# YuePanEdward/GH-ICP

Measured on AMD Instinct MI355X. Metric: registered_pairs_per_sec, higher is better.
Workload: dtype f64

## Files before the change

### gh-icp_amd/csrc/batch.hip

```cpp
#include "batch_dev.h"
#include "frontend.h"
#include "pca_dev.h"
#include "bsc_dev.h"
#include "prims.h"

#include <cmath>

namespace {

enum { FB_CLOUD_BY_CLOUD = -1, FB_HALVE = -2 };

__global__ void k_fb_bbox_init(int* __restrict__ bb, int nb) {
  const int i = blockIdx.x * 256 + threadIdx.x;
  if (i < nb * 6) bb[i] = (i % 6) < 3 ? 0x7f7fffff : (int)0x80800000;
}

__global__ __launch_bounds__(256) void k_fb_bbox(const FbBlock* __restrict__ D, const float* __restrict__ base, int which, int* __restrict__ bb) {
  __shared__ float smin[3][4], smax[3][4];
  const int b = blockIdx.y;
  const float* xyz;
  long long n;
  int stride;
  if (which == 0) { xyz = D->c[b].xyz; n = D->c[b].n; stride = D->c[b].stride; }
  else {
// ... 178 lines not shown
  const int b = fb_find(D->moff, D->nb, i);
  D->c[b].ds[i - D->moff[b]] = dsg[i];
}

__global__ __launch_bounds__(256) void k_fb_keypoints_out(const FbBlock* __restrict__ D, const float4* __restrict__ dsg, const int* __restrict__ kpg, int K,
                                                          float* __restrict__ lcs) {
  const int t = blockIdx.x * 256 + threadIdx.x;
  if (t >= K) return;
  const int b = fb_find(D->koff, D->nb, t), j = t - D->koff[b];
  const int id = kpg[D->coff[b] + j];
  const float4 P = dsg[D->moff[b] + id];
  const FbCloud& C = D->c[b];
  C.kp[j] = id;
  C.kpx[(size_t)j * 3] = (double)P.x; C.kpx[(size_t)j * 3 + 1] = (double)P.y; C.kpx[(size_t)j * 3 + 2] = (double)P.z;
  if (lcs) { lcs[(size_t)t * 12 + 9] = P.x; lcs[(size_t)t * 12 + 10] = P.y; lcs[(size_t)t * 12 + 11] = P.z; }
}

__global__ __launch_bounds__(256) void k_fb_zero_feat(const FbBlock* __restrict__ D, int K) {
  const int t = blockIdx.x * 256 + threadIdx.x;
  if (t >= K * 56) return;
  const int q = t / 56, r = t % 56, v = r / 14, w = r % 14;
  const int b = fb_find(D->koff, D->nb, q), j = q - D->koff[b], kb = D->koff[b + 1] - D->koff[b];
  reinterpret_cast<unsigned*>(D->c[b].feat)[((size_t)v * kb + j) * 14 + w] = 0u;
}

__global__ __launch_bounds__(256) void k_fb_gather_rows33(const FbBlock* __restrict__ D, const float* __restrict__ hist, int K) {
  const int t = blockIdx.x * 256 + threadIdx.x;
  if (t >= K * 33) return;
  const int q = t / 33, r = t % 33;
  const int b = fb_find(D->koff, D->nb, q), j = q - D->koff[b];
  reinterpret_cast<float*>(D->c[b].feat)[(size_t)j * 33 + r] = hist[((size_t)D->moff[b] + D->c[b].kp[j]) * 33 + r];
}

__global__ __launch_bounds__(BT) void k_fb_bsc(const FbBlock* __restrict__ D, const float4* __restrict__ pts, const unsigned* __restrict__ start, BscConst C,
                                               float* __restrict__ lcs) {
  const int q = blockIdx.x;
  const int b = fb_find(D->koff, D->nb, q);
  GridArgs G;
  G.d = D->g2[b]; G.pts = pts; G.start = start + D->cb2[b];
  gh_bsc_keypoint(G, C, q - D->koff[b], D->koff[b + 1] - D->koff[b], D->c[b].feat, lcs + (size_t)D->koff[b] * 12);
}

void decode_box(const int* enc, float* mm) {
  for (int k = 0; k < 6; k++) {
    const int i = enc[k] >= 0 ? enc[k] : enc[k] ^ 0x7fffffff;
    memcpy(&mm[k], &i, 4);
  }
}

int build_grid(ghicp_ctx* ctx, const FbBlock* D, int which, const float4* dsg, int M, unsigned total_cells, const GridSlots& sl, const float4** pts_out,
               const unsigned** start_out, const unsigned** keys_out) {
  hipStream_t s = ctx->stream;
  unsigned *keys, *keys2, *vals, *vals2, *start;
  float4* pts;
  GH_TRY(ctx->reserve(sl.keys, (size_t)M + 1, &keys));
  GH_TRY(ctx->reserve(sl.keys2, (size_t)M + 1, &keys2));
  GH_TRY(ctx->reserve(sl.vals, (size_t)M + 1, &vals));
  GH_TRY(ctx->reserve(sl.vals2, (size_t)M + 1, &vals2));
  GH_TRY(ctx->reserve(sl.start, (size_t)total_cells + 2, &start));
  GH_TRY(ctx->reserve(sl.pts, (size_t)M + 1, &pts));
  hipEvent_t kg = ctx->kt_begin(KT_FB_GRID);
  hipLaunchKernelGGL(k_fb_cell_keys, dim3(cdiv(M, 256)), dim3(256), 0, s, D, which, dsg, M, keys, vals);
  GH_TRY(gh_radix_sort_u32(ctx, keys, keys2, vals, vals2, M, 0, bits_for(total_cells)));
  hipLaunchKernelGGL(k_fb_gather_sorted, dim3(cdiv(M, 256)), dim3(256), 0, s, dsg, vals2, M, pts);
  gh_cell_start_launch(s, keys2, (unsigned)M, total_cells, start);
  ctx->kt_end(KT_FB_GRID, kg);
  GH_HIP(hipGetLastError());
  *pts_out = pts; *start_out = start; *keys_out = keys2;
  return GHICP_OK;
}

int fb_cloud_by_cloud(int n_clouds, ghicp_cloud* const* clouds, const float* const* xyz, const int64_t* n, int stride) {
  for (int i = 0; i < n_clouds; i++) GH_TRY(ghicp_cloud_recompute(clouds[i], xyz[i], n[i], stride));
// ... 172 lines not shown
  for (int b = 0; b < nb; b++) clouds[b]->cand = H->coff[b + 1] - H->coff[b];
  Ctot = H->coff[nb];
  return GHICP_OK;
}

int FbRun::outputs() {
  for (int b = 0; b < nb; b++) {
    ghicp_cloud* c = clouds[b];
    GH_HIP(c->ds.reserve(((size_t)c->m + 1) * sizeof(float4)));
    GH_HIP(c->kp.reserve(((size_t)c->m + 1) * sizeof(int)));
    GH_HIP(c->kpx.reserve(((size_t)c->k * 3 + 3) * sizeof(double)));
    if (bsc) GH_HIP(c->feat.reserve((size_t)4 * c->k * 56 + 64));
    if (fpfh) GH_HIP(c->feat.reserve(((size_t)c->k * 33 + 33) * sizeof(float)));
    H->c[b].ds = c->ds.as<float4>(); H->c[b].kp = c->kp.as<int>(); H->c[b].kpx = c->kpx.as<double>(); H->c[b].feat = c->feat.as<uint8_t>();
  }
  GH_HIP(upload());
  hipEvent_t ko = ctx->kt_begin(KT_FB_OUT);
  hipLaunchKernelGGL(k_fb_copy_ds, dim3(cdiv(M, 256)), dim3(256), 0, s, (const FbBlock*)D, (const float4*)dsg, M);
  lcs = nullptr;
  if (Ktot > 0) {
    if (bsc) GH_TRY(ctx->reserve(B_P_LCS, (size_t)Ktot * 12 + 12, &lcs));
    hipLaunchKernelGGL(k_fb_keypoints_out, dim3(cdiv(Ktot, 256)), dim3(256), 0, s, (const FbBlock*)D, (const float4*)dsg, (const int*)kpg, Ktot, lcs);
    if (bsc) hipLaunchKernelGGL(k_fb_zero_feat, dim3(cdiv((long long)Ktot * 56, 256)), dim3(256), 0, s, (const FbBlock*)D, Ktot);
  }
  ctx->kt_end(KT_FB_OUT, ko);
  return GHICP_OK;
}

int FbRun::features(const BscConst& BC) {
  if (Ktot > 0 && (bsc || fpfh)) {
    const float4* pts2;
    const unsigned *start2, *keys2;
    const GridSlots sl2 = {B_GRID2_KEYS, B_GRID2_KEYS2, B_GRID2_VALS, B_GRID2_VALS2, B_GRID2_START, B_GRID2_PTS};
    GH_TRY(build_grid(ctx, D, 1, dsg, M, (unsigned)t2, sl2, &pts2, &start2, &keys2));
    if (bsc) {
      hipEvent_t kb = ctx->kt_begin(KT_BSC);
      hipLaunchKernelGGL(k_fb_bsc, dim3((unsigned)Ktot), dim3(BT), 0, s, (const FbBlock*)D, pts2, start2, BC, lcs);
      ctx->kt_end(KT_BSC, kb);
    } else {
      float* hist;
      GH_TRY(ctx->reserve(B_P_FEAT_S, (size_t)M * 33 * sizeof(float) + 64, (char**)&hist));
      GH_TRY(gh_fpfh_batch_dev(ctx, dsg, M, pts2, start2, D->g2, D->cb2, D->moff, nb, hist));
      hipLaunchKernelGGL(k_fb_gather_rows33, dim3(cdiv((long long)Ktot * 33, 256)), dim3(256), 0, s, (const FbBlock*)D, (const float*)hist, Ktot);
    }
  }
  GH_HIP(hipGetLastError());
  GH_HIP(hipStreamSynchronize(s));
  return GHICP_OK;
}

extern "C" int ghicp_clouds_recompute(ghicp_ctx* ctx, int32_t n_clouds, ghicp_cloud* const* clouds, const float* const* xyz, const int64_t* n, int stride) {
  GH_ENTER(ctx);
  GH_ARG(n_clouds >= 0 && (n_clouds == 0 || (clouds != nullptr && xyz != nullptr && n != nullptr)) && stride >= 3);
  if (n_clouds == 0) return GHICP_OK;
  FbRun R;
  R.ctx = ctx; R.s = ctx->stream; R.nb = n_clouds; R.clouds = clouds; R.N = 0;
  for (int i = 0; i < n_clouds; i++) {
    GH_ARG(clouds[i] != nullptr && clouds[i]->ctx == ctx && n[i] >= 0 && n[i] < (1ll << 31) - 2);
    if (!same_front_end(clouds[i]->cfg, clouds[0]->cfg))
      return ctx->fail(GHICP_ERR_ARG, "ghicp_clouds_recompute: cloud %d has a different front-end configuration", i);
    for (int j = 0; j < i; j++) GH_ARG(clouds[j] != clouds[i]);
    R.N += n[i];
  }
  R.cfg = clouds[0]->cfg; R.bsc = R.cfg.reg.feature == GHICP_FEATURE_BSC; R.fpfh = R.cfg.reg.feature == GHICP_FEATURE_FPFH;
  if (!(R.cfg.voxel > 0.f) || ctx->host_ptrs) return fb_cloud_by_cloud(n_clouds, clouds, xyz, n, stride);
  if (n_clouds > FB_MAX || R.N + n_clouds >= (1ll << 31) - 2) return fb_halve(ctx, n_clouds, clouds, xyz, n, stride);
  GH_TRY(R.begin(xyz, n, stride));
  if (R.N == 0) return GHICP_OK;
  BscConst BC;
  int rc = R.raw_boxes();
  if (rc == GHICP_OK) rc = R.voxel();
// ... 10 lines not shown
```

### gh-icp_amd/csrc/bsc.hip

```cpp
#include "frontend.h"
#include "devmath.h"
#include "bsc_dev.h"

namespace {

__global__ __launch_bounds__(BT) void k_bsc(GridArgs G, const int* __restrict__ kp, BscConst C, uint8_t* __restrict__ feat, float* __restrict__ lcs) {
  gh_bsc_keypoint(G, C, (int)blockIdx.x, C.K, feat, lcs);
}

__global__ __launch_bounds__(256) void k_bsc_origins(const float* __restrict__ xyz, int stride, const int* __restrict__ kp, int K, float* __restrict__ lcs) {
  const int k = blockIdx.x * 256 + threadIdx.x;
  if (k >= K) return;
  const long long s = kp[k];
  lcs[(size_t)k * 12 + 9] = xyz[s * stride];
  lcs[(size_t)k * 12 + 10] = xyz[s * stride + 1];
  lcs[(size_t)k * 12 + 11] = xyz[s * stride + 2];
}

}

int gh_bsc_make_const(ghicp_ctx* ctx, float R, int dof, const int32_t* pattern_host, BscConst* out, float* r_search) {
  BscConst C;
  memset(&C, 0, sizeof(C));
  C.R = R;
  const double rs = std::sqrt(3.0) * (double)R;
  C.r2s = (float)(rs * rs);
  C.u = 2 * R / 7;
  const float delta = (float)(C.u * 0.5);
  C.den = 2 * delta * delta;
  C.r2c = (float)((1.5 * (double)C.u) * (1.5 * (double)C.u));
  C.area = (float)(M_PI * (double)R * (double)R);
  C.radius_w = std::sqrt(2.0) * (double)R;
  int ex = 0;
  (void)std::frexp((double)R * 0.5, &ex);
  C.dunit = std::ldexp(1.0, 24 - ex);
  C.dinv = std::ldexp(1.0, ex - 54);
  for (int i = 0; i < 7; i++) C.centre[i] = (float)((i + 0.5) * (double)C.u - (double)R);
  for (int i = 0; i < 98; i++) {
    C.pattern[i] = pattern_host[i];
    if (C.pattern[i] < 0 || C.pattern[i] > 48) return ctx->fail(GHICP_ERR_ARG, "BSC sample pattern entry %d out of [0,48]", i);
  }
  C.K = 0;
  C.nvar = (dof > 4) ? 4 : (dof > 0 ? 2 : 1);
  *out = C;
  *r_search = (float)rs;
  return GHICP_OK;
}

int gh_bsc_dev(ghicp_ctx* ctx, const float* xyz, long long m, int stride, const int32_t* kp, long long K, float R, int dof, const int32_t* pattern_host,
               uint8_t* feat, float* lcs) {
  if (K <= 0) return GHICP_OK;
  hipStream_t s = ctx->stream;
  BscConst C;
  float r_search_f = 0.f;
  GH_TRY(gh_bsc_make_const(ctx, R, dof, pattern_host, &C, &r_search_f));
  C.K = (int)K;
  DeviceGrid G;
  const GridSlots sl = {B_GRID2_KEYS, B_GRID2_KEYS2, B_GRID2_VALS, B_GRID2_VALS2, B_GRID2_START, B_GRID2_PTS};
  GH_TRY(gh_grid_build(ctx, xyz, m, stride, r_search_f * 1.0001f, sl, &G));
  GH_HIP(hipMemsetAsync(feat, 0, (size_t)4 * K * 56, s));
  hipLaunchKernelGGL(k_bsc_origins, dim3(cdiv(K, 256)), dim3(256), 0, s, xyz, stride, kp, (int)K, lcs);
  GridArgs A = {G.d, G.pts, G.start};
  hipEvent_t kt = ctx->kt_begin(KT_BSC);
  hipLaunchKernelGGL(k_bsc, dim3((unsigned)K), dim3(BT), 0, s, A, kp, C, feat, lcs);
  ctx->kt_end(KT_BSC, kt);
  GH_HIP(hipGetLastError());
  return GHICP_OK;
}

extern "C" int ghicp_bsc_encode(ghicp_ctx* ctx, const float* xyz, int64_t m, int stride, const int32_t* kp_idx, int64_t k, float radius, int dof,
                                const int32_t* pattern, uint8_t* feat, float* lcs) {
  GH_ENTER(ctx);
  GH_ARG(m >= 0 && m < (1ll << 31) - 2 && k >= 0 && k <= m && stride >= 3 && radius > 0.f && pattern != nullptr);
  Stager sg(ctx);
  const float* d;
  const int32_t* dk;
  uint8_t* df;
  float* dl;
  GH_TRY(sg.in_cloud(xyz, (size_t)m * stride, &d));
  GH_TRY(sg.in(kp_idx, (size_t)k, &dk));
  GH_TRY(sg.out(feat, (size_t)4 * k * 56, &df));
  GH_TRY(sg.out(lcs, (size_t)k * 12, &dl));
  GH_TRY(gh_bsc_dev(ctx, d, m, stride, dk, k, radius, dof, pattern, df, dl));
  return sg.finish();
}
```

### gh-icp_amd/csrc/bsc_dev.h

```cpp
#pragma once
#include "grid.h"
#include "devmath.h"
#include "bsc_exp_table.h"

struct BscConst {
  float R, r2s, u, den, r2c, area;
  double radius_w;
  double dunit, dinv;
  float centre[7];
  int pattern[98];
  int K, nvar;
};

constexpr int BT = 256;
constexpr int BSC_CAP = 2048;
constexpr int BSC_CHUNK = 512;

int gh_bsc_make_const(ghicp_ctx* ctx, float R, int dof, const int32_t* pattern_host, BscConst* out, float* r_search);

static __device__ const double gh_bsc_exp_tab[145] = {GH_BSC_EXP_TABLE};
__device__ inline float gh_bsc_expf(float xf, const double* __restrict__ tab) {
  const double x = (double)xf;
  int j = (int)(x * -32.0 + 0.5);
  j = j < 0 ? 0 : (j > 144 ? 144 : j);
  const double s = x + (double)j * 0.03125;
  double p = s * (1.0 / 720.0) + (1.0 / 120.0);
  p = s * p + (1.0 / 24.0);
  p = s * p + (1.0 / 6.0);
  p = s * p + 0.5;
  p = s * p + 1.0;
  p = s * p + 1.0;
  return (float)(tab[j] * p);
}

__device__ inline void gh_bsc_depth_add(unsigned long long* __restrict__ lo64, unsigned* __restrict__ carry, float depth, float ew, double dunit) {
  const unsigned d_off = (unsigned)((int)((double)depth * dunit) + (1 << 27));
  const unsigned w_int = (unsigned)((double)ew * 1073741824.0);
  const unsigned long long term = (unsigned long long)d_off * (unsigned long long)w_int;
  const unsigned long long old = atomicAdd(lo64, term);
  if (old + term < old) atomicAdd(carry, 1u);
}
__device__ inline double gh_bsc_depth_sum(unsigned long long lo64, unsigned carry, double pnum, double dinv) {
  const unsigned __int128 acc = ((unsigned __int128)carry << 64) | (unsigned __int128)lo64;
  const unsigned __int128 shift = (unsigned __int128)(unsigned long long)(pnum * 1073741824.0) << 27;
  const bool neg = acc < shift;
  const unsigned __int128 mag = neg ? shift - acc : acc - shift;
  const double d = (double)(unsigned long long)(mag >> 32) * 4294967296.0 + (double)(unsigned long long)(mag & 0xFFFFFFFFull);
  return (neg ? -d : d) * dinv;
}

__device__ inline int rearr_src(int type, int k) {
  switch (type) {
    case 1: return 48 - k;
    case 2: return (6 - k / 7) * 7 + k % 7;
    default: return (k / 7) * 7 + 6 - k % 7;
  }
}

__device__ inline void gh_bsc_keypoint(const GridArgs& G, const BscConst& C, int kk, int K, uint8_t* __restrict__ feat, float* __restrict__ lcs) {

  __shared__ double red[16];
  __shared__ double s_pnum[147], s_exp[145];
  __shared__ unsigned long long s_dlo[147];
  __shared__ unsigned s_dcarry[147];
  __shared__ float s_weight[147], s_depth[147];
  __shared__ float s_axes[9];
  __shared__ double s_stat[3][4];
  __shared__ unsigned s_bits[4][16];
  __shared__ float4 s_pts[BSC_CHUNK];
  __shared__ int s_scan[17];
  __shared__ float s_centre[8];
  const int tid = threadIdx.x;
  const float qx = lcs[(size_t)kk * 12 + 9], qy = lcs[(size_t)kk * 12 + 10], qz = lcs[(size_t)kk * 12 + 11];
  const int cx = gh_cell_coord(qx, G.d.mn[0], G.d.inv, G.d.dim[0]);
  const int cy = gh_cell_coord(qy, G.d.mn[1], G.d.inv, G.d.dim[1]);
  const int cz = gh_cell_coord(qz, G.d.mn[2], G.d.inv, G.d.dim[2]);

  double sx = 0, sy = 0, sz = 0, sw = 0;
  int cnt = 0;
  gh_for_runs(G.d, G.start, cx, cy, cz, [&](unsigned b, unsigned e) {
    for (unsigned q = b + tid; q < e; q += BT) {
      const float4 P = G.pts[q];
      const float dx = qx - P.x, dy = qy - P.y, dz = qz - P.z;
      float d2 = dx * dx;
      d2 += dy * dy;
      d2 += dz * dz;
      if (d2 < C.r2s) {
        cnt++;
        sx += (double)P.x; sy += (double)P.y; sz += (double)P.z;
        sw += C.radius_w - (double)sqrtf(d2);
      }
    }
  });
  sx = gh_block_sum(sx, red); sy = gh_block_sum(sy, red); sz = gh_block_sum(sz, red); sw = gh_block_sum(sw, red);
  int mm;
  const int my_base = gh_block_excl_scan(cnt, s_scan, &mm);
  const double mx = sx / (double)mm, my = sy / (double)mm, mz = sz / (double)mm;
  const bool packed = mm <= BSC_CAP;
  auto fill_chunk = [&](int c0) {
    int w = my_base;
    gh_for_runs(G.d, G.start, cx, cy, cz, [&](unsigned b, unsigned e) {
      for (unsigned q = b + tid; q < e; q += BT) {
        const float4 P = G.pts[q];
        const float dx = qx - P.x, dy = qy - P.y, dz = qz - P.z;
        float d2 = dx * dx;
        d2 += dy * dy;
        d2 += dz * dz;
        if (d2 < C.r2s) {
          if (w >= c0 && w < c0 + BSC_CHUNK) s_pts[w - c0] = make_float4(P.x, P.y, P.z, d2);
          w++;
        }
      }
    });
    __syncthreads();
  };

  double c00 = 0, c01 = 0, c02 = 0, c11 = 0, c12 = 0, c22 = 0;
  if (mm >= 3 && packed) {
    for (int c0 = 0; c0 < mm; c0 += BSC_CHUNK) {
      fill_chunk(c0);
      const int cn = min(BSC_CHUNK, mm - c0);
      for (int t = tid; t < cn; t += BT) {
        const float4 P = s_pts[t];
        const double w = (double)(float)(C.radius_w - (double)sqrtf(P.w));
        const double ex = (double)P.x - mx, ey = (double)P.y - my, ez = (double)P.z - mz;
        c00 += w * ex * ex; c01 += w * ex * ey; c02 += w * ex * ez;
        c11 += w * ey * ey; c12 += w * ey * ez; c22 += w * ez * ez;
      }
      __syncthreads();
    }
  } else if (mm >= 3) {
    gh_for_runs(G.d, G.start, cx, cy, cz, [&](unsigned b, unsigned e) {
      for (unsigned q = b + tid; q < e; q += BT) {
        const float4 P = G.pts[q];
        const float dx = qx - P.x, dy = qy - P.y, dz = qz - P.z;
        float d2 = dx * dx;
        d2 += dy * dy;
        d2 += dz * dz;
        if (d2 < C.r2s) {
          const double w = (double)(float)(C.radius_w - (double)sqrtf(d2));
          const double ex = (double)P.x - mx, ey = (double)P.y - my, ez = (double)P.z - mz;
          c00 += w * ex * ex; c01 += w * ex * ey; c02 += w * ex * ez;
          c11 += w * ey * ey; c12 += w * ey * ez; c22 += w * ez * ez;
        }
      }
    });
  }
  if (mm >= 3) {
    c00 = gh_block_sum(c00, red); c01 = gh_block_sum(c01, red); c02 = gh_block_sum(c02, red);
    c11 = gh_block_sum(c11, red); c12 = gh_block_sum(c12, red); c22 = gh_block_sum(c22, red);
  }
  if (tid == 0) {
    float X[3] = {1, 0, 0}, Y[3] = {0, 1, 0}, Z[3] = {0, 0, 1};
    if (mm >= 3) {
      const float da = (float)sw;
      double Cq[6] = {c00, c01, c02, c11, c12, c22};
      gh_quant_grid(Cq, 6);
      double a00 = (double)((float)Cq[0] / da), a01 = (double)((float)Cq[1] / da), a02 = (double)((float)Cq[2] / da),
             a11 = (double)((float)Cq[3] / da), a12 = (double)((float)Cq[4] / da), a22 = (double)((float)Cq[5] / da);
      double V[9];
      gh_jacobi3(a00, a01, a02, a11, a12, a22, V);
      const double ev[3] = {a00, a11, a22};
      int imax = 0, imin = 0;
// ... 1 lines not shown
        if ((float)ev[i] > (float)ev[imax]) imax = i;
        if ((float)ev[i] < (float)ev[imin]) imin = i;
      }
      float P[3], N[3];
      for (int which = 0; which < 2; which++) {
        const int col = which == 0 ? imax : imin;
        const double e[3] = {V[0 * 3 + col], V[1 * 3 + col], V[2 * 3 + col]};
        int b = 0;
        if (fabs(e[1]) > fabs(e[b])) b = 1;
        if (fabs(e[2]) > fabs(e[b])) b = 2;
        const double sg = (e[b] < 0) ? -1.0 : 1.0;
        float* o = which == 0 ? P : N;
        for (int d = 0; d < 3; d++) o[d] = (float)(sg * e[d]);
      }
      const float M0 = P[1] * N[2] - P[2] * N[1], M1 = P[2] * N[0] - P[0] * N[2], M2 = P[0] * N[1] - P[1] * N[0];
      X[0] = P[0]; X[1] = P[1]; X[2] = P[2];
      Y[0] = M0; Y[1] = M1; Y[2] = M2;
      Z[0] = X[1] * Y[2] - X[2] * Y[1];
      Z[1] = X[2] * Y[0] - X[0] * Y[2];
      Z[2] = X[0] * Y[1] - X[1] * Y[0];
      const float nx = sqrtf((X[0] * X[0] + X[1] * X[1]) + X[2] * X[2]);
      const float ny = sqrtf((Y[0] * Y[0] + Y[1] * Y[1]) + Y[2] * Y[2]);
      for (int d = 0; d < 3; d++) { X[d] = X[d] / nx; Y[d] = Y[d] / ny; }
    }
    for (int d = 0; d < 3; d++) { s_axes[d] = X[d]; s_axes[3 + d] = Y[d]; s_axes[6 + d] = Z[d]; }
    float* o = &lcs[(size_t)kk * 12];
    for (int d = 0; d < 3; d++) { o[d] = X[d]; o[3 + d] = Y[d]; o[6 + d] = Z[d]; }
  }
  for (int i = tid; i < 147; i += BT) { s_pnum[i] = 0.0; s_dlo[i] = 0ull; s_dcarry[i] = 0u; }
  for (int i = tid; i < 145; i += BT) s_exp[i] = gh_bsc_exp_tab[i];
  if (tid < 7) s_centre[tid] = C.centre[tid];
  if (tid < 64) s_bits[tid >> 4][tid & 15] = 0u;
  __syncthreads();
  const float X0 = s_axes[0], X1 = s_axes[1], X2 = s_axes[2], Y0 = s_axes[3], Y1 = s_axes[4], Y2 = s_axes[5], Z0 = s_axes[6], Z1 = s_axes[7],
              Z2 = s_axes[8];

  auto splat = [&](float px, float py, float pz) {
    const float d0 = px - qx, d1 = py - qy, d2v = pz - qz;
    const float loc[3] = {(X0 * d0 + X1 * d1) + X2 * d2v, (Y0 * d0 + Y1 * d1) + Y2 * d2v, (Z0 * d0 + Z1 * d1) + Z2 * d2v};
#pragma unroll
    for (int pl = 0; pl < 3; pl++) {
      const float a = loc[pl == 2 ? 1 : 0], bb = loc[pl == 0 ? 1 : 2];
      const float depth = loc[pl == 0 ? 2 : (pl == 1 ? 1 : 0)] + C.R;
      for (int j = 0; j < 7; j++) {
        const float dy = bb - C.centre[j];
        const float dy2 = dy * dy;
        if (!(dy2 < C.r2c)) continue;
        for (int i = 0; i < 7; i++) {
          const float dx = a - C.centre[i];
          float dd = dx * dx;
          dd += dy2;
          if (dd < C.r2c) {
            const float ew = gh_bsc_expf(-dd / C.den, s_exp);
            atomicAdd(&s_pnum[i + 7 * j + 49 * pl], (double)ew);
            gh_bsc_depth_add(&s_dlo[i + 7 * j + 49 * pl], &s_dcarry[i + 7 * j + 49 * pl], depth, ew, C.dunit);
          }
        }
      }
    }
  };
  if (packed) {
    const int wave = tid >> 6, lane = tid & 63;
    const int sub = lane / 9, slot = lane % 9;
    const int di = slot % 3 - 1, dj = slot / 3 - 1;
    const float inv_u = 1.0f / C.u;
    for (int c0 = 0; c0 < mm; c0 += BSC_CHUNK) {
    fill_chunk(c0);
    const int cn = min(BSC_CHUNK, mm - c0);
    for (int t = tid; t < cn; t += BT) {
      const float4 P = s_pts[t];
      const float d0 = P.x - qx, d1 = P.y - qy, d2v = P.z - qz;
      s_pts[t] = make_float4((X0 * d0 + X1 * d1) + X2 * d2v, (Y0 * d0 + Y1 * d1) + Y2 * d2v, (Z0 * d0 + Z1 * d1) + Z2 * d2v, 0.f);
    }
    __syncthreads();
    const int nitem = cn * 3;
    for (int base = 0; base < nitem; base += 28) {
      const int w = base + wave * 7 + sub;
      if (lane < 63 && w < nitem) {
        const int t = w / 3, pl = w - 3 * t;
        const float4 L = s_pts[t];
        const float a = pl == 2 ? L.y : L.x, bb = pl == 0 ? L.y : L.z;
        const float depth = (pl == 0 ? L.z : (pl == 1 ? L.y : L.x)) + C.R;
        const float ta = (a + C.R) * inv_u, tb = (bb + C.R) * inv_u;
        const float fla = floorf(ta), flb = floorf(tb);
        const int bi = (int)fla, bj = (int)flb;
        auto cell = [&](int ci, int cj) {
          if (ci < 0 || ci >= 7 || cj < 0 || cj >= 7) return;
          const float dy = bb - s_centre[cj];
          const float dy2 = dy * dy;
          const float dx = a - s_centre[ci];
          float dd = dx * dx;
          dd += dy2;
          if (dy2 < C.r2c && dd < C.r2c) {
            const float ew = gh_bsc_expf(-dd / C.den, s_exp);
            atomicAdd(&s_pnum[ci + 7 * cj + 49 * pl], (double)ew);
            gh_bsc_depth_add(&s_dlo[ci + 7 * cj + 49 * pl], &s_dcarry[ci + 7 * cj + 49 * pl], depth, ew, C.dunit);
          }
        };
        cell(bi + di, bj + dj);
        const float fa = ta - fla, fb = tb - flb;
        if (fa < 1e-4f || fa > 0.9999f || fb < 1e-4f || fb > 0.9999f) {
          bool fx = false, fy = false;
          const int i2 = bi + 2 * di, j2 = bj + 2 * dj;
          if (di != 0 && i2 >= 0 && i2 < 7) { const float dx = a - s_centre[i2]; fx = dx * dx < C.r2c; }
          if (dj != 0 && j2 >= 0 && j2 < 7) { const float dy = bb - s_centre[j2]; fy = dy * dy < C.r2c; }
          if (fx) cell(i2, bj + dj);
          if (fy) cell(bi + di, j2);
          if (fx && fy) cell(i2, j2);
        }
      }
    }
    __syncthreads();
    }
  } else {
    gh_for_runs(G.d, G.start, cx, cy, cz, [&](unsigned b, unsigned e) {
      for (unsigned q = b + tid; q < e; q += BT) {
        const float4 P = G.pts[q];
        const float tx = qx - P.x, ty = qy - P.y, tz = qz - P.z;
        float d2 = tx * tx;
        d2 += ty * ty;
        d2 += tz * tz;
        if (!(d2 < C.r2s)) continue;
        splat(P.x, P.y, P.z);
      }
    });
  }
  __syncthreads();

  if (tid < 147) {
    const float ndens = (float)mm / C.area;
    float avg = (float)gh_bsc_depth_sum(s_dlo[tid], s_dcarry[tid], s_pnum[tid], C.dinv);
    avg = (s_pnum[tid] == 0.0) ? 0.0f : (float)((double)avg / s_pnum[tid]);
    const float garea = C.u * C.u;
    const float gdens = (float)(s_pnum[tid] / (double)garea);
    s_weight[tid] = (ndens != 0.0f) ? gdens / ndens : 0.0f;
    s_depth[tid] = avg;
  }
  __syncthreads();
  if (tid < 3) {
    const int off = 49 * tid;
    double avg_d = 0, var_d = 0, avg_w = 0, var_w = 0;
    for (int i = 0; i < 49; i++) {
      const int a = C.pattern[2 * i] + off, b = C.pattern[2 * i + 1] + off;
      avg_d += (double)(s_depth[a] - s_depth[b]);
      avg_w += (double)(s_weight[a] - s_weight[b]);
    }
    avg_d /= 49; avg_w /= 49;
    for (int i = 0; i < 49; i++) {
      const int a = C.pattern[2 * i] + off, b = C.pattern[2 * i + 1] + off;
      const double dd = (double)(s_depth[a] - s_depth[b]), dw = (double)(s_weight[a] - s_weight[b]);
      var_d += (dd - avg_d) * (dd - avg_d);
      var_w += (dw - avg_w) * (dw - avg_w);
    }
    var_d /= 49; var_w /= 49;
    s_stat[tid][0] = avg_d; s_stat[tid][1] = sqrt(var_d); s_stat[tid][2] = avg_w; s_stat[tid][3] = sqrt(var_w);
  }
  __syncthreads();
  for (int base = 0; base < 448; base += BT) {
    const int k = base + tid;
    for (int v = 0; v < C.nvar; v++) {
      bool bit = false;
      if (v == 0) {
        if (k < 147) bit = s_weight[k] > 0.1f;
        else if (k < 441) {
          const int r = k - 147, pl = r / 98, p = (r % 98) >> 1, off = 49 * pl;
          const int a = C.pattern[2 * p], b = C.pattern[2 * p + 1];
          if ((r & 1) == 0) {
            const double dd = (double)(s_depth[a + off] - s_depth[b + off]);
            bit = fabs(dd - s_stat[pl][0]) > s_stat[pl][1];
          } else if (!(s_weight[a] < 0.1f && s_weight[b] < 0.1f)) {
            const double dw = (double)(s_weight[a + off] - s_weight[b + off]);
            bit = fabs(dw - s_stat[pl][2]) > s_stat[pl][3];
          }
        }
      } else if (k >= 147 && k < 294) {
        static const int TR[4][3] = {{0, 0, 0}, {1, 2, 2}, {3, 2, 1}, {2, 1, 3}};
        const int r = k - 147, pl = r / 49, kk2 = r % 49;
        bit = s_weight[49 * pl + rearr_src(TR[v][pl], kk2)] > 0.1f;
      }
      const unsigned long long bal = __ballot(bit);
      if ((tid & 63) == 0 && k < 448) {
        s_bits[v][k >> 5] = (unsigned)bal;
        if (k + 32 < 448) s_bits[v][(k >> 5) + 1] = (unsigned)(bal >> 32);
      }
    }
  }
  __syncthreads();
  if (tid < 14 * C.nvar) {
    const int v = tid / 14, w = tid % 14;
    reinterpret_cast<unsigned*>(feat)[((size_t)v * K + kk) * 14 + w] = s_bits[v][w];
  }
}
```

### gh-icp_amd/csrc/ctx.h

```cpp
#pragma once
#include <hip/hip_runtime.h>

#include <atomic>
#include <cstdarg>
#include <cstdio>
#include <cstring>
#include <string>
#include <vector>

#include "../../include/ghicp_c.h"

#define GH_HIP(call)                                                                                          \
  do {                                                                                                        \
    hipError_t e_ = (call);                                                                                   \
    if (e_ != hipSuccess) return ctx->fail(GHICP_ERR_HIP, "%s:%d %s -> %s", __FILE__, __LINE__, #call, hipGetErrorString(e_)); \
  } while (0)
#define GH_TRY(call)               \
  do {                             \
    int r_ = (call);               \
    if (r_ != GHICP_OK) return r_; \
  } while (0)
#define GH_ARG(cond)                                                                \
  do {                                                                              \
    if (!(cond)) return ctx->fail(GHICP_ERR_ARG, "%s: bad argument (%s)", __func__, #cond); \
// ... 13 lines not shown
    if (p) {
      hipError_t e = hipFree(p);
      if (e != hipSuccess) return e;
      p = nullptr; cap = 0;
    }
    size_t want = bytes + bytes / 4 + 256;
    hipError_t e = hipMalloc(&p, want);
    if (e != hipSuccess) return e;
    cap = want;
    return hipSuccess;
  }
  template <typename T> T* as() const { return reinterpret_cast<T*>(p); }
  void release() { if (p) (void)hipFree(p); p = nullptr; cap = 0; }
};

enum BufSlot {
  B_LOOP_STATE = 0, B_LOOP_SP, B_LOOP_KMW, B_LOOP_KMSCR,
  B_GRID_KEYS, B_GRID_KEYS2, B_GRID_VALS, B_GRID_VALS2, B_GRID_TMP, B_GRID_START, B_GRID_PTS, B_GRID_MISC,
  B_GRID2_KEYS, B_GRID2_KEYS2, B_GRID2_VALS, B_GRID2_VALS2, B_GRID2_START, B_GRID2_PTS,
  B_FE_LAMBDA, B_FE_CURV, B_FE_COUNT, B_FE_CAND, B_FE_STATE, B_FE_KP, B_FE_SORTK, B_FE_SORTK2, B_FE_SORTV, B_FE_SORTV2, B_FE_CPTS,
  B_FE_FLAGS, B_FE_SCAN, B_FE_SCATTER,
  B_P_KEEP_S, B_P_KEEP_T, B_P_DS_S, B_P_DS_T, B_P_KP_S, B_P_KP_T, B_P_KPXYZ_S, B_P_KPXYZ_T, B_P_FEAT_S, B_P_FEAT_T, B_P_LCS,
  B_P_FD, B_P_MISC, B_P_PATTERN, B_FD_JOBS, B_TRANSFORM_JOBS,
  B_KM_LX, B_KM_MISC, B_KM_SLACK, B_KM_LSTAT, B_KM_ORDER, B_KM_MASK,
  B_FB_DESC, B_FB_HEADPOS, B_FB_DS,
  B_PRIM_TMP, B_NMSR_KEY, B_NMSR_CELL, B_NMSR_TABLE, B_NMSR_HEAD, B_NMSR_PTS, B_NMSR_SKEY, B_NMSR_STATE, B_NMSR_NEXT, B_NMSR_SEL, B_NMSR_LIST, B_NMSR_PTS0, B_NMSR_SKEY0,
  B_ICP_TC_KEYS, B_ICP_TC_KEYS2, B_ICP_TC_VALS, B_ICP_TC_VALS2, B_ICP_TC_START, B_ICP_TC_PTS,
  B_ICP_SC_KEYS, B_ICP_SC_KEYS2, B_ICP_SC_VALS, B_ICP_SC_VALS2, B_ICP_SC_START, B_ICP_SC_PTS,
  B_ICP_CUR, B_ICP_Q, B_ICP_NN, B_ICP_ND, B_ICP_NN2, B_ICP_ND2, B_ICP_KEYS, B_ICP_PART, B_ICP_STATE,
  B_ICP_PEND, B_ICP_TNRM, B_ICP_OUT,
  B_GICP_COVS, B_GICP_COVT, B_GICP_MAHAL, B_GICP_SRC4,
  B_SOR_DIST, B_SOR_PART,
  B_RF_DESC, B_RF_MISC,
  B_NUM
};

enum KtSlot { KT_PCA = 0, KT_BSC, KT_KM_SOLVE, KT_CD_ROWMIN, KT_KM_WEIGHTS, KT_FD_BSC, KT_NMS_ROUND, KT_VOXEL_SORT,
              KT_FB_VOXEL, KT_FB_GRID, KT_FB_PRUNE, KT_FB_RANK, KT_FB_OUT,
              KT_PAIR_LOOP,
              KT_TRANSFORM,
              KT_PAIR_LOOP_DISPATCH,
              KT_REFINE,
              KT_GICP_CLOUDS,
              KT_NUM };
static const char* const kKtNames[KT_NUM] = {"pca_cells", "bsc", "km_solve", "cd_rowmin", "km_weights", "fd_bsc", "nms_round", "voxel_sort",
                                             "fb_voxel", "fb_grid", "fb_prune", "fb_rank", "fb_out", "pair_loop", "transform", "pair_loop_dispatch", "refine", "gicp_clouds"};

struct ghicp_ctx {
  bool kt_on = false;
  double kt_ms[KT_NUM] = {0};
  long long kt_count[KT_NUM] = {0};
  struct KtPending { int slot; hipEvent_t a, b; };
  std::vector<KtPending> kt_pending;
  std::vector<hipEvent_t> kt_pool;
  hipEvent_t kt_event() {
    if (!kt_pool.empty()) { hipEvent_t e = kt_pool.back(); kt_pool.pop_back(); return e; }
    hipEvent_t e = nullptr;
    (void)hipEventCreate(&e);
    return e;
  }
  hipEvent_t kt_begin(int slot) { return kt_begin_on(slot, stream); }
  void kt_end(int slot, hipEvent_t a) { kt_end_on(slot, a, stream); }
  hipEvent_t kt_begin_on(int slot, hipStream_t st) {
    if (!kt_on) return nullptr;
    hipEvent_t a = kt_event();
    (void)hipEventRecord(a, st);
// ... 13 lines not shown
      kt_pool.push_back(p.a);
      kt_pool.push_back(p.b);
    }
    kt_pending.clear();
  }
  static constexpr int KM_LSTAT_MAX = 8192;
  static constexpr int KM_LSTAT_W = 12;
  long long km_launches = 0;
  std::vector<int> km_slots;
  long long loop_hazards = 0;
  std::vector<float> loop_cost_hints;
  std::vector<long long> loop_timeline;
  std::atomic<long long> loop_active{0}, loop_total{0};
  bool bbox_valid = false;
  const float* bbox_ptr = nullptr;
  long long bbox_n = 0;
  int bbox_stride = 0;
  float bbox_mm[6] = {0, 0, 0, 0, 0, 0};
  int device = 0;
  hipStream_t stream = nullptr;
  hipStream_t own_stream = nullptr;
  bool km_stats = false, km_force_hazard = false;
  int loop_slots_cap = 0;
  bool loop_confine = true;
  double loop_confine_margin = 1.15;
  hipStream_t confine_stream = nullptr, rest_stream = nullptr;
  int confine_cus = 0;
  struct ConfinePair { int cus; hipStream_t confined, rest; };
  std::vector<ConfinePair> confine_cache;
  bool km_compact = true;
  int km_compact_from = 0;
  int km_kflags() const { return (km_force_hazard ? 4 : 0) | (km_compact_from << 8); }
  bool loop_fuse = true;
  int loop_min_lds = 0;
  std::vector<uint32_t> cu_mask;
  std::vector<hipStream_t> aux_streams;
  std::vector<hipEvent_t> aux_events;
  int* progress_host = nullptr;
  std::atomic<bool> progress_live{false};
  bool host_ptrs = false;
  struct Staged { const void* host; size_t bytes; uint64_t fp; void* dev; uint64_t tick; };
  std::vector<Staged> staged;
  size_t staged_bytes = 0;
  uint64_t stage_tick = 0;
  long long staged_hits = 0, staged_misses = 0;
  void stage_clear() {
    if (staged.empty()) return;
    (void)hipStreamSynchronize(stream);
    for (auto& e : staged) (void)hipFree(e.dev);
    staged.clear();
    staged_bytes = 0;
  }
  static constexpr size_t STAGED_MIN = 256 * 1024, STAGED_CAP = (size_t)1 << 30;
  std::string err;
  DevBuf buf[B_NUM];
  std::vector<DevBuf> pairbuf;
  void* pinned = nullptr;
  void* job_pinned = nullptr;
  size_t job_pinned_cap = 0;
  hipEvent_t job_event = nullptr;
  bool job_pending = false;
  int upload_table(const void* src, size_t bytes, void* dst) {
    if (job_pending) {
      if (hipEventSynchronize(job_event) != hipSuccess) return fail(GHICP_ERR_HIP, "job table: event wait failed");
      job_pending = false;
    }
// ... 162 lines not shown
```

### gh-icp_amd/csrc/ctx.hip

```cpp
#include "ctx.h"
#include "devmath.h"

extern "C" const char* ghicp_version(void) { return "ghicp-hip 0.1 (gfx950)"; }

extern "C" void ghicp_params_default(ghicp_params* p) {
  if (!p) return;
  memset(p, 0, sizeof(*p));
  p->feature = GHICP_FEATURE_BSC;
  p->corr = GHICP_CORR_KM;
  p->dof = 6;
  p->max_iter = 200;
  p->radius_nonmax = 1.5f;
  p->adjust_ratio = 1.1f;
  p->adjust_step = 0.1f;
  p->est_iou = 0.6f;
  p->converge_t = 0.02f;
  p->converge_r = 0.02f;
  p->bbx_magnitude = 0.f;
  p->penalty_initial = 2.0;
  p->para1 = 1.0;
  p->para2 = 1.0;
  p->km_eps = 0.01;
  p->min_cor = 10;
  p->weight_changing_rate = 6;
}

extern "C" int ghicp_ctx_create(int device, ghicp_ctx** out) {
  if (!out) return GHICP_ERR_ARG;
  *out = nullptr;
  int count = 0;
  if (hipGetDeviceCount(&count) != hipSuccess || count <= 0 || device < 0 || device >= count) return GHICP_ERR_NO_GPU;
  if (hipSetDevice(device) != hipSuccess) return GHICP_ERR_NO_GPU;
  hipDeviceProp_t prop;
  if (hipGetDeviceProperties(&prop, device) != hipSuccess) return GHICP_ERR_NO_GPU;
  ghicp_ctx* c = new ghicp_ctx();
  c->device = device;
  c->num_cu = prop.multiProcessorCount > 0 ? prop.multiProcessorCount : 256;
  c->km_stats = getenv("GHICP_KM_STATS") != nullptr;
  c->km_force_hazard = getenv("GHICP_KM_FORCE_HAZARD") != nullptr;
  if (const char* e = getenv("GHICP_LOOP_SLOTS")) c->loop_slots_cap = atoi(e) > 0 ? atoi(e) : 0;
  if (const char* e = getenv("GHICP_LOOP_CONFINE")) c->loop_confine = atoi(e) != 0;
  if (const char* e = getenv("GHICP_KM_COMPACT")) c->km_compact = atoi(e) != 0;
  if (const char* e = getenv("GHICP_LOOP_FUSE")) c->loop_fuse = atoi(e) != 0;
  if (const char* e = getenv("GHICP_KM_COMPACT_FROM")) c->km_compact_from = atoi(e) > 0 && atoi(e) < 65535 ? atoi(e) : 0;
  if (const char* e = getenv("GHICP_LOOP_MIN_LDS")) c->loop_min_lds = atoi(e) > 0 ? atoi(e) : 0;
  if (const char* e = getenv("GHICP_LOOP_CONFINE_MARGIN")) { const double m = atof(e); if (m >= 0.25 && m <= 4.0) c->loop_confine_margin = m; }
  if (hipHostMalloc(&c->pinned, 4096, hipHostMallocDefault) != hipSuccess) { delete c; return GHICP_ERR_HIP; }
  c->pinned_cap = 4096;
  *out = c;
  return GHICP_OK;
}

extern "C" int ghicp_ctx_destroy(ghicp_ctx* ctx) {
  if (!ctx) return GHICP_OK;
  (void)hipSetDevice(ctx->device);
  (void)hipDeviceSynchronize();
  ctx->kt_collect();
  for (hipEvent_t e : ctx->kt_pool) (void)hipEventDestroy(e);
  for (ghicp_cloud* c : ctx->pair_clouds) (void)ghicp_cloud_destroy(c);
  ctx->pair_clouds.clear();
  for (int i = 0; i < B_NUM; i++) ctx->buf[i].release();
  for (auto& b : ctx->pairbuf) b.release();
  ctx->stage_clear();
  if (ctx->pinned) (void)hipHostFree(ctx->pinned);
  if (ctx->job_pinned) (void)hipHostFree(ctx->job_pinned);
  if (ctx->job_event) (void)hipEventDestroy(ctx->job_event);
  if (ctx->fb_pinned) (void)hipHostFree(ctx->fb_pinned);
  if (ctx->own_stream) (void)hipStreamDestroy(ctx->own_stream);
  for (auto& e : ctx->confine_cache) { (void)hipStreamDestroy(e.confined); (void)hipStreamDestroy(e.rest); }
  for (hipStream_t a : ctx->aux_streams) (void)hipStreamDestroy(a);
  for (hipEvent_t e : ctx->aux_events) (void)hipEventDestroy(e);
  if (ctx->progress_host) (void)hipHostFree(ctx->progress_host);
  delete ctx;
  return GHICP_OK;
}

extern "C" int ghicp_ctx_stage_stats(const ghicp_ctx* ctx, int64_t* hits, int64_t* misses, int64_t* bytes_kept) {
// ... 379 lines not shown
```

Before: 425.1.

## Spill BSC neighbour points to global slots instead of re-gathering per chunk

For keypoints whose neighbourhood exceeds the shared-memory chunk, the BSC kernel used to re-walk the grid and refill shared memory for every chunk, in both the covariance pass and the voxel pass. Points are now gathered once into a per-block global spill slot, claimed from a pool sized by occupancy with an atomic flag, and read back from there. This removes the repeated grid traversal at the cost of extra global traffic, an atomic slot claim and a memset per launch. Optional cycle-counter profiling, enabled by an environment variable, is compiled in as a template variant.

```diff
diff --git a/gh-icp_amd/csrc/batch.hip b/gh-icp_amd/csrc/batch.hip
--- a/gh-icp_amd/csrc/batch.hip
+++ b/gh-icp_amd/csrc/batch.hip
@@ -234,13 +234,14 @@
   reinterpret_cast<float*>(D->c[b].feat)[(size_t)j * 33 + r] = hist[((size_t)D->moff[b] + D->c[b].kp[j]) * 33 + r];
 }
 
+template <bool PROF>
 __global__ __launch_bounds__(BT) void k_fb_bsc(const FbBlock* __restrict__ D, const float4* __restrict__ pts, const unsigned* __restrict__ start, BscConst C,
-                                               float* __restrict__ lcs) {
+                                               float* __restrict__ lcs, BscSpill W) {
   const int q = blockIdx.x;
   const int b = fb_find(D->koff, D->nb, q);
   GridArgs G;
   G.d = D->g2[b]; G.pts = pts; G.start = start + D->cb2[b];
-  gh_bsc_keypoint(G, C, q - D->koff[b], D->koff[b + 1] - D->koff[b], D->c[b].feat, lcs + (size_t)D->koff[b] * 12);
+  gh_bsc_keypoint<PROF>(G, C, q - D->koff[b], D->koff[b + 1] - D->koff[b], D->c[b].feat, lcs + (size_t)D->koff[b] * 12, W);
 }
 
 void decode_box(const int* enc, float* mm) {
@@ -479,11 +480,20 @@
     const float4* pts2;
     const unsigned *start2, *keys2;
     const GridSlots sl2 = {B_GRID2_KEYS, B_GRID2_KEYS2, B_GRID2_VALS, B_GRID2_VALS2, B_GRID2_START, B_GRID2_PTS};
+    BscSpill W;
+    if (bsc) {
+      int per_cu = 0;
+      GH_HIP(hipOccupancyMaxActiveBlocksPerMultiprocessor(&per_cu, reinterpret_cast<const void*>(&k_fb_bsc<false>), BT, 0));
+      GH_TRY(gh_bsc_spill_reserve(ctx, Ktot, per_cu, &W));
+    }
     GH_TRY(build_grid(ctx, D, 1, dsg, M, (unsigned)t2, sl2, &pts2, &start2, &keys2));
     if (bsc) {
+      GH_TRY(gh_bsc_spill_begin(ctx, W));
       hipEvent_t kb = ctx->kt_begin(KT_BSC);
-      hipLaunchKernelGGL(k_fb_bsc, dim3((unsigned)Ktot), dim3(BT), 0, s, (const FbBlock*)D, pts2, start2, BC, lcs);
+      if (ctx->bsc_stats) hipLaunchKernelGGL(k_fb_bsc<true>, dim3((unsigned)Ktot), dim3(BT), 0, s, (const FbBlock*)D, pts2, start2, BC, lcs, W);
+      else hipLaunchKernelGGL(k_fb_bsc<false>, dim3((unsigned)Ktot), dim3(BT), 0, s, (const FbBlock*)D, pts2, start2, BC, lcs, W);
       ctx->kt_end(KT_BSC, kb);
+      GH_TRY(gh_bsc_spill_report(ctx, W, "k_fb_bsc", Ktot));
     } else {
       float* hist;
       GH_TRY(ctx->reserve(B_P_FEAT_S, (size_t)M * 33 * sizeof(float) + 64, (char**)&hist));
diff --git a/gh-icp_amd/csrc/bsc.hip b/gh-icp_amd/csrc/bsc.hip
--- a/gh-icp_amd/csrc/bsc.hip
+++ b/gh-icp_amd/csrc/bsc.hip
@@ -4,8 +4,9 @@
 
 namespace {
 
-__global__ __launch_bounds__(BT) void k_bsc(GridArgs G, const int* __restrict__ kp, BscConst C, uint8_t* __restrict__ feat, float* __restrict__ lcs) {
-  gh_bsc_keypoint(G, C, (int)blockIdx.x, C.K, feat, lcs);
+template <bool PROF>
+__global__ __launch_bounds__(BT) void k_bsc(GridArgs G, BscConst C, uint8_t* __restrict__ feat, float* __restrict__ lcs, BscSpill W) {
+  gh_bsc_keypoint<PROF>(G, C, (int)blockIdx.x, C.K, feat, lcs, W);
 }
 
 __global__ __launch_bounds__(256) void k_bsc_origins(const float* __restrict__ xyz, int stride, const int* __restrict__ kp, int K, float* __restrict__ lcs) {
@@ -47,6 +48,35 @@
   return GHICP_OK;
 }
 
+int gh_bsc_spill_reserve(ghicp_ctx* ctx, long long K, int per_cu, BscSpill* out) {
+  long long n = (long long)std::max(1, per_cu) * std::max(1, ctx->num_cu);
+  if (ctx->bsc_slots_cap > 0) n = std::min<long long>(n, ctx->bsc_slots_cap);
+  n = std::max<long long>(1, std::min(n, K));
+  const size_t head = 64 + (((size_t)n * sizeof(unsigned) + 255) & ~(size_t)255);
+  char* base;
+  GH_TRY(ctx->reserve(B_BSC_SPILL, head + (size_t)n * BSC_CAP * sizeof(float4), &base));
+  out->nslots = (int)n;
+  out->prof = reinterpret_cast<unsigned long long*>(base);
+  out->flags = reinterpret_cast<unsigned*>(base + 64);
+  out->slots = reinterpret_cast<float4*>(base + head);
+  return GHICP_OK;
+}
+
+int gh_bsc_spill_begin(ghicp_ctx* ctx, const BscSpill& g) {
+  GH_HIP(hipMemsetAsync(g.prof, 0, 64 + (size_t)g.nslots * sizeof(unsigned), ctx->stream));
+  return GHICP_OK;
+}
+
+int gh_bsc_spill_report(ghicp_ctx* ctx, const BscSpill& g, const char* kernel, long long K) {
+  if (!ctx->bsc_stats) return GHICP_OK;
+  unsigned long long h[BSC_PROF_W];
+  GH_HIP(hipMemcpyAsync(h, g.prof, sizeof(h), hipMemcpyDeviceToHost, ctx->stream));
+  GH_HIP(hipStreamSynchronize(ctx->stream));
+  fprintf(stderr, "bsc_stats %s keypoints %lld slots %d cycles: count %llu place %llu cov %llu to_lcs %llu items %llu tail %llu | taken %llu total %llu\n", kernel, K, g.nslots,
+          h[0], h[1], h[2], h[3], h[4], h[5], h[6], h[7]);
+  return GHICP_OK;
+}
+
 int gh_bsc_dev(ghicp_ctx* ctx, const float* xyz, long long m, int stride, const int32_t* kp, long long K, float R, int dof, const int32_t* pattern_host,
                uint8_t* feat, float* lcs) {
   if (K <= 0) return GHICP_OK;
@@ -57,15 +87,21 @@
   C.K = (int)K;
   DeviceGrid G;
   const GridSlots sl = {B_GRID2_KEYS, B_GRID2_KEYS2, B_GRID2_VALS, B_GRID2_VALS2, B_GRID2_START, B_GRID2_PTS};
+  int per_cu = 0;
+  GH_HIP(hipOccupancyMaxActiveBlocksPerMultiprocessor(&per_cu, reinterpret_cast<const void*>(&k_bsc<false>), BT, 0));
+  BscSpill W;
+  GH_TRY(gh_bsc_spill_reserve(ctx, K, per_cu, &W));
   GH_TRY(gh_grid_build(ctx, xyz, m, stride, r_search_f * 1.0001f, sl, &G));
   GH_HIP(hipMemsetAsync(feat, 0, (size_t)4 * K * 56, s));
   hipLaunchKernelGGL(k_bsc_origins, dim3(cdiv(K, 256)), dim3(256), 0, s, xyz, stride, kp, (int)K, lcs);
   GridArgs A = {G.d, G.pts, G.start};
   hipEvent_t kt = ctx->kt_begin(KT_BSC);
-  hipLaunchKernelGGL(k_bsc, dim3((unsigned)K), dim3(BT), 0, s, A, kp, C, feat, lcs);
+  GH_TRY(gh_bsc_spill_begin(ctx, W));
+  if (ctx->bsc_stats) hipLaunchKernelGGL(k_bsc<true>, dim3((unsigned)K), dim3(BT), 0, s, A, C, feat, lcs, W);
+  else hipLaunchKernelGGL(k_bsc<false>, dim3((unsigned)K), dim3(BT), 0, s, A, C, feat, lcs, W);
   ctx->kt_end(KT_BSC, kt);
   GH_HIP(hipGetLastError());
-  return GHICP_OK;
+  return gh_bsc_spill_report(ctx, W, "k_bsc", K);
 }
 
 extern "C" int ghicp_bsc_encode(ghicp_ctx* ctx, const float* xyz, int64_t m, int stride, const int32_t* kp_idx, int64_t k, float radius, int dof,
diff --git a/gh-icp_amd/csrc/bsc_dev.h b/gh-icp_amd/csrc/bsc_dev.h
--- a/gh-icp_amd/csrc/bsc_dev.h
+++ b/gh-icp_amd/csrc/bsc_dev.h
@@ -17,6 +17,16 @@
 constexpr int BSC_CHUNK = 512;
 
 int gh_bsc_make_const(ghicp_ctx* ctx, float R, int dof, const int32_t* pattern_host, BscConst* out, float* r_search);
+
+struct BscSpill {
+  int nslots;
+  unsigned* flags;
+  unsigned long long* prof;
+  float4* slots;
+};
+int gh_bsc_spill_reserve(ghicp_ctx* ctx, long long K, int per_cu, BscSpill* out);
+int gh_bsc_spill_begin(ghicp_ctx* ctx, const BscSpill& g);
+int gh_bsc_spill_report(ghicp_ctx* ctx, const BscSpill& g, const char* kernel, long long K);
 
 static __device__ const double gh_bsc_exp_tab[145] = {GH_BSC_EXP_TABLE};
 __device__ inline float gh_bsc_expf(float xf, const double* __restrict__ tab) {
@@ -57,7 +67,34 @@
   }
 }
 
-__device__ inline void gh_bsc_keypoint(const GridArgs& G, const BscConst& C, int kk, int K, uint8_t* __restrict__ feat, float* __restrict__ lcs) {
+constexpr int BSC_PROF_W = 8;
+template <bool PROF>
+struct BscClock {
+  long long t;
+  unsigned long long* acc;
+  __device__ inline BscClock(unsigned long long* a) : t(PROF ? (long long)__builtin_readcyclecounter() : 0), acc(a) {}
+  __device__ inline void lap(int stage) {
+    if (!PROF) return;
+    const long long x = (long long)__builtin_readcyclecounter();
+    if (threadIdx.x == 0) atomicAdd(&acc[stage], (unsigned long long)(x - t));
+    t = x;
+  }
+};
+
+__device__ inline int gh_bsc_slot_claim(const BscSpill& W) {
+  __shared__ int s_slot;
+  if (threadIdx.x == 0) {
+    int i = (int)(blockIdx.x % (unsigned)W.nslots);
+    while (atomicCAS(&W.flags[i], 0u, 1u) != 0u) i = i + 1 == W.nslots ? 0 : i + 1;
+    s_slot = i;
+  }
+  __syncthreads();
+  return s_slot;
+}
+
+template <bool PROF>
+__device__ inline void gh_bsc_keypoint(const GridArgs& G, const BscConst& C, int kk, int K, uint8_t* __restrict__ feat, float* __restrict__ lcs,
+                                       const BscSpill& W) {
 
   __shared__ double red[16];
   __shared__ double s_pnum[147], s_exp[145];
@@ -71,6 +108,8 @@
   __shared__ int s_scan[17];
   __shared__ float s_centre[8];
   const int tid = threadIdx.x;
+  BscClock<PROF> clk(W.prof);
+  const long long t_kp = clk.t;
   const float qx = lcs[(size_t)kk * 12 + 9], qy = lcs[(size_t)kk * 12 + 10], qz = lcs[(size_t)kk * 12 + 11];
   const int cx = gh_cell_coord(qx, G.d.mn[0], G.d.inv, G.d.dim[0]);
   const int cy = gh_cell_coord(qy, G.d.mn[1], G.d.inv, G.d.dim[1]);
@@ -97,7 +136,11 @@
   const int my_base = gh_block_excl_scan(cnt, s_scan, &mm);
   const double mx = sx / (double)mm, my = sy / (double)mm, mz = sz / (double)mm;
   const bool packed = mm <= BSC_CAP;
-  auto fill_chunk = [&](int c0) {
+  const bool resident = mm <= BSC_CHUNK;
+  clk.lap(0);
+  const int held = (packed && !resident) ? gh_bsc_slot_claim(W) : -1;
+  float4* spill = W.slots + (size_t)(held < 0 ? 0 : held) * BSC_CAP;
+  if (packed) {
     int w = my_base;
     gh_for_runs(G.d, G.start, cx, cy, cz, [&](unsigned b, unsigned e) {
       for (unsigned q = b + tid; q < e; q += BT) {
@@ -107,28 +150,26 @@
         d2 += dy * dy;
         d2 += dz * dz;
         if (d2 < C.r2s) {
-          if (w >= c0 && w < c0 + BSC_CHUNK) s_pts[w - c0] = make_float4(P.x, P.y, P.z, d2);
+          if (resident) s_pts[w] = make_float4(P.x, P.y, P.z, d2);
+          else spill[w] = make_float4(P.x, P.y, P.z, d2);
           w++;
         }
       }
     });
     __syncthreads();
-  };
+  }
+  clk.lap(1);
 
   double c00 = 0, c01 = 0, c02 = 0, c11 = 0, c12 = 0, c22 = 0;
   if (mm >= 3 && packed) {
-    for (int c0 = 0; c0 < mm; c0 += BSC_CHUNK) {
-      fill_chunk(c0);
-      const int cn = min(BSC_CHUNK, mm - c0);
-      for (int t = tid; t < cn; t += BT) {
-        const float4 P = s_pts[t];
-        const double w = (double)(float)(C.radius_w - (double)sqrtf(P.w));
-        const double ex = (double)P.x - mx, ey = (double)P.y - my, ez = (double)P.z - mz;
-        c00 += w * ex * ex; c01 += w * ex * ey; c02 += w * ex * ez;
-        c11 += w * ey * ey; c12 += w * ey * ez; c22 += w * ez * ez;
-      }
-      __syncthreads();
-    }
+    auto scatter = [&](const float4 P) {
+      const double w = (double)(float)(C.radius_w - (double)sqrtf(P.w));
+      const double ex = (double)P.x - mx, ey = (double)P.y - my, ez = (double)P.z - mz;
+      c00 += w * ex * ex; c01 += w * ex * ey; c02 += w * ex * ez;
+      c11 += w * ey * ey; c12 += w * ey * ez; c22 += w * ez * ez;
+    };
+    if (resident) for (int t = tid; t < mm; t += BT) scatter(s_pts[t]);
+    else for (int t = tid; t < mm; t += BT) scatter(spill[t]);
   } else if (mm >= 3) {
     gh_for_runs(G.d, G.start, cx, cy, cz, [&](unsigned b, unsigned e) {
       for (unsigned q = b + tid; q < e; q += BT) {
@@ -196,6 +237,7 @@
   if (tid < 7) s_centre[tid] = C.centre[tid];
   if (tid < 64) s_bits[tid >> 4][tid & 15] = 0u;
   __syncthreads();
+  clk.lap(2);
   const float X0 = s_axes[0], X1 = s_axes[1], X2 = s_axes[2], Y0 = s_axes[3], Y1 = s_axes[4], Y2 = s_axes[5], Z0 = s_axes[6], Z1 = s_axes[7],
               Z2 = s_axes[8];
 
@@ -229,14 +271,14 @@
     const int di = slot % 3 - 1, dj = slot / 3 - 1;
     const float inv_u = 1.0f / C.u;
     for (int c0 = 0; c0 < mm; c0 += BSC_CHUNK) {
-    fill_chunk(c0);
     const int cn = min(BSC_CHUNK, mm - c0);
     for (int t = tid; t < cn; t += BT) {
-      const float4 P = s_pts[t];
+      const float4 P = resident ? s_pts[t] : spill[c0 + t];
       const float d0 = P.x - qx, d1 = P.y - qy, d2v = P.z - qz;
       s_pts[t] = make_float4((X0 * d0 + X1 * d1) + X2 * d2v, (Y0 * d0 + Y1 * d1) + Y2 * d2v, (Z0 * d0 + Z1 * d1) + Z2 * d2v, 0.f);
     }
     __syncthreads();
+    clk.lap(3);
     const int nitem = cn * 3;
     for (int base = 0; base < nitem; base += 28) {
       const int w = base + wave * 7 + sub;
@@ -275,7 +317,9 @@
       }
     }
     __syncthreads();
-    }
+    clk.lap(4);
+    }
+    if (held >= 0 && tid == 0) atomicExch(&W.flags[held], 0u);
   } else {
     gh_for_runs(G.d, G.start, cx, cy, cz, [&](unsigned b, unsigned e) {
       for (unsigned q = b + tid; q < e; q += BT) {
@@ -290,6 +334,7 @@
     });
   }
   __syncthreads();
+  clk.lap(4);
 
   if (tid < 147) {
     const float ndens = (float)mm / C.area;
@@ -354,4 +399,6 @@
     const int v = tid / 14, w = tid % 14;
     reinterpret_cast<unsigned*>(feat)[((size_t)v * K + kk) * 14 + w] = s_bits[v][w];
   }
-}
+  clk.lap(5);
+  if (PROF && tid == 0) { atomicAdd(&W.prof[6], 1ull); atomicAdd(&W.prof[7], (unsigned long long)(clk.t - t_kp)); }
+}
diff --git a/gh-icp_amd/csrc/ctx.h b/gh-icp_amd/csrc/ctx.h
--- a/gh-icp_amd/csrc/ctx.h
+++ b/gh-icp_amd/csrc/ctx.h
@@ -69,6 +69,7 @@
   B_GICP_COVS, B_GICP_COVT, B_GICP_MAHAL, B_GICP_SRC4,
   B_SOR_DIST, B_SOR_PART,
   B_RF_DESC, B_RF_MISC,
+  B_BSC_SPILL,
   B_NUM
 };
 
@@ -148,6 +149,8 @@
   int km_compact_from = 0;
   int km_kflags() const { return (km_force_hazard ? 4 : 0) | (km_compact_from << 8); }
   bool loop_fuse = true;
+  bool bsc_stats = false;
+  int bsc_slots_cap = 0;
   int loop_min_lds = 0;
   std::vector<uint32_t> cu_mask;
   std::vector<hipStream_t> aux_streams;
diff --git a/gh-icp_amd/csrc/ctx.hip b/gh-icp_amd/csrc/ctx.hip
--- a/gh-icp_amd/csrc/ctx.hip
+++ b/gh-icp_amd/csrc/ctx.hip
@@ -43,6 +43,8 @@
   if (const char* e = getenv("GHICP_KM_COMPACT")) c->km_compact = atoi(e) != 0;
   if (const char* e = getenv("GHICP_LOOP_FUSE")) c->loop_fuse = atoi(e) != 0;
   if (const char* e = getenv("GHICP_KM_COMPACT_FROM")) c->km_compact_from = atoi(e) > 0 && atoi(e) < 65535 ? atoi(e) : 0;
+  c->bsc_stats = getenv("GHICP_BSC_STATS") != nullptr;
+  if (const char* e = getenv("GHICP_BSC_SLOTS")) c->bsc_slots_cap = atoi(e) > 0 ? atoi(e) : 0;
   if (const char* e = getenv("GHICP_LOOP_MIN_LDS")) c->loop_min_lds = atoi(e) > 0 ? atoi(e) : 0;
   if (const char* e = getenv("GHICP_LOOP_CONFINE_MARGIN")) { const double m = atof(e); if (m >= 0.25 && m <= 4.0) c->loop_confine_margin = m; }
   if (hipHostMalloc(&c->pinned, 4096, hipHostMallocDefault) != hipSuccess) { delete c; return GHICP_ERR_HIP; }
```

After: 427.2 (median of 6 runs). About the same (+0.5%).
